# bjg-gh/style_transfer_visualizer

Hardware: AMD Instinct MI355X
Metric: optimization steps/sec at 512² and 1024², 1/2/4/8 MI355X (higher is better)
Workload: dtype bf16; 1 GPU; single 512x512 image per GPU, L-BFGS (max_iter=1, history 100), VGG19 bf16 storage / fp32 accumulate, fp32 Gram, --no-video (BASELINE.json configs[1]); weights: synthetic He-scaled; size=512, images=1, init_method=random, parallelism=replicas x1 (independent images), lbfgs_history_prefill_steps=95, world_size=1

## Files before the change

### style_transfer_visualizer_amd/csrc/conv_igemm_kernel.h

```cpp
#pragma once
#include <type_traits>
#include <utility>

#include "stv_common.h"
#include "conv_args.h"
#include "conv_tiles.h"

#ifndef STV_STAMP
#define STV_STAMP(k) do {} while (0)
#endif
#ifndef STV_DIAG
#define STV_DIAG 0
#endif

#ifndef STV_HOLD_LAST
#define STV_HOLD_LAST 1
#endif
#ifndef STV_X_AUX
#define STV_X_AUX 0
#endif
#ifndef STV_STORE_AUX
#define STV_STORE_AUX 0
#endif

extern thread_local const void* g_stv_next_w;
extern thread_local uint32_t g_stv_next_w_bytes;

namespace {


template <typename T, int TH_, int BN_, int WM_, int WN_, int TAPS_, int KS_ = 1, int NBUF_ = 3, bool M16_ = false,
          bool X3_ = false>
struct Cfg {
  static constexpr bool X3 = X3_;
  static constexpr bool M16 = M16_;
  using Elem = T;
  static constexpr int TH = TH_, BN = BN_, WM = WM_, WN = WN_, TAPS = TAPS_;
  static constexpr int NWAVES = WM_ * WN_;
  static constexpr int KS = KS_;
  static constexpr int GT = 64 * NWAVES;
  static constexpr int TW = 32;
  static constexpr int KB = 32;
  static constexpr int CK = KB / (int)sizeof(T);
  static constexpr int HALO = (TAPS == 9) ? 1 : 0;
  static constexpr int ND = (TAPS == 9) ? 3 : 1;
  static constexpr int IN_H = TH + 2 * HALO, IN_W = TW + 2 * HALO;
  static constexpr int IN_PIX = IN_H * IN_W;
  static constexpr int W_ROWS = TAPS * BN;
  static constexpr int MT = TH / WM;
  static constexpr int NT = BN / WN / 32;
  static constexpr int AROWS = MT + 2 * HALO;
  static constexpr bool BIG = MT * NT >= 8;
  static constexpr int THREADS = GT * KS;
  static constexpr int IN_PIECES = (IN_PIX * 2 + 63) / 64;
  static constexpr int W_PIECES = (W_ROWS * 2 + 63) / 64;
  static constexpr int PIECES = IN_PIECES + W_PIECES;
  static constexpr int PPW = (PIECES + NWAVES - 1) / NWAVES;
  static constexpr int IN_BYTES = IN_PIECES * 1024;
  static constexpr int SPARE_OFF = PIECES * 1024;
  static constexpr int STAGE_BYTES = SPARE_OFF + 1024;
  static constexpr int NBUF = NBUF_;
  static constexpr int BM = TH * TW;
  static constexpr int CS = BN + 4;
  static constexpr int C_BYTES = BM * CS * 4;
  static constexpr int RING_BYTES = NBUF * KS * STAGE_BYTES;
  static constexpr int LDS_BYTES = (KS == 1 || RING_BYTES > C_BYTES) ? RING_BYTES : C_BYTES;
  static_assert(NWAVES * KS == 4 || NWAVES * KS == 8, "4 or 8 waves per workgroup");
  static_assert(KS == 1 || KS == 2, "K split");
  static_assert(NBUF >= 2 && NBUF <= 6, "ring depth");
  static_assert(!M16 || (NBUF == 4 && sizeof(T) == 2), "16x16x32 main loop: bf16, two pairs of stage slots");
  static_assert(!X3 || (sizeof(T) == 4 && !M16), "split-bf16 products: fp32 storage, 32x32 main loop");
  static_assert(TH % WM == 0 && BN % (WN * 32) == 0, "tile split");
  static_assert(BN % 16 == 0, "swizzle period");
  static_assert(LDS_BYTES <= 160 * 1024, "LDS budget");
};

template <typename T> struct Frag;
template <> struct Frag<bf16_t> { using type = bf16x8v; };
template <> struct Frag<float> { using type = f32x4; };

template <typename T>
__device__ __forceinline__ void mma(const typename Frag<T>::type& a,
                                    const typename Frag<T>::type& b, f32x16& acc);
template <>
__device__ __forceinline__ void mma<bf16_t>(const bf16x8v& a, const bf16x8v& b, f32x16& acc) {
  acc = __builtin_amdgcn_mfma_f32_32x32x16_bf16(a, b, acc, 0, 0, 0);
}
template <>
__device__ __forceinline__ void mma<float>(const f32x4& a, const f32x4& b, f32x16& acc) {
#pragma unroll
  for (int j = 0; j < 4; ++j) acc = __builtin_amdgcn_mfma_f32_32x32x2f32(a[j], b[j], acc, 0, 0, 0);
}

struct X3Act { bf16x8v p, q; };

__device__ __forceinline__ float bf16_hi_part(float x, uint32_t& bits) {
  bits = (uint32_t)f32_to_bf16(x);
  return __uint_as_float(bits << 16);
}
__device__ __forceinline__ void split4(f32x4 v, uint32_t (&hi)[2], uint32_t (&lo)[2]) {
#pragma unroll
  for (int i = 0; i < 2; ++i) {
    uint32_t b0, b1;
    const float h0 = bf16_hi_part(v[2 * i], b0), h1 = bf16_hi_part(v[2 * i + 1], b1);
    const float r0 = __builtin_isfinite(h0) ? v[2 * i] - h0 : 0.0f;
    const float r1 = __builtin_isfinite(h1) ? v[2 * i + 1] - h1 : 0.0f;
    hi[i] = b0 | (b1 << 16);
    lo[i] = pack_bf16x2(r0, r1);
  }
}
__device__ __forceinline__ X3Act split_act(f32x4 v) {
  uint32_t hi[2], lo[2];
  split4(v, hi, lo);
  const u32x4 p = {hi[0], hi[1], hi[0], hi[1]}, q = {lo[0], lo[1], 0u, 0u};
  return X3Act{__builtin_bit_cast(bf16x8v, p), __builtin_bit_cast(bf16x8v, q)};
}
__device__ __forceinline__ bf16x8v split_w(f32x4 v) {
  uint32_t hi[2], lo[2];
  split4(v, hi, lo);
  const u32x4 w = {hi[0], hi[1], lo[0], lo[1]};
  return __builtin_bit_cast(bf16x8v, w);
}
__device__ __forceinline__ void mma_any(const f32x4& b, const f32x4& a, f32x16& acc) { mma<float>(b, a, acc); }
__device__ __forceinline__ void mma_any(const bf16x8v& b, const bf16x8v& a, f32x16& acc) { mma<bf16_t>(b, a, acc); }
__device__ __forceinline__ void mma_any(const bf16x8v& w, const X3Act& a, f32x16& acc) {
  acc = __builtin_amdgcn_mfma_f32_32x32x16_bf16(w, a.p, acc, 0, 0, 0);
  acc = __builtin_amdgcn_mfma_f32_32x32x16_bf16(w, a.q, acc, 0, 0, 0);
}

template <typename T>
struct Phase {
  const T* x;
  const T* w;
  int cin;
  bool w_blocked;
};
struct Geom {
  int H, W, cout, x0, y0, n0;
  int lane, wave, grp, wm, wn, r, h;
};

template <typename C, bool RELU>
__device__ __forceinline__ void conv_mainloop(const Phase<typename C::Elem>& ph, const Geom& gm, char* smem,
                                              f32x16 (&acc)[C::MT][C::NT]) {
  using T = typename C::Elem;
  using FragT = typename Frag<T>::type;
  using AFrag = std::conditional_t<C::X3, X3Act, FragT>;
  using BFrag = std::conditional_t<C::X3, bf16x8v, FragT>;
  using lds_ptr = __attribute__((address_space(3))) void*;
  constexpr int kVec = elem_traits<T>::kVec;
  const int lane = gm.lane, wave = gm.wave, grp = gm.grp, wm = gm.wm, wn = gm.wn, r = gm.r, h = gm.h;
  const int x0 = gm.x0, y0 = gm.y0, n0 = gm.n0;
  const int nchunks = ph.cin / C::CK;
  constexpr uint32_t kOob = 0x80000000u;
  const int x_bytes = gm.H * gm.W * ph.cin * (int)sizeof(T);
  const int w_bytes = C::TAPS * gm.cout * ph.cin * (int)sizeof(T);
  const int w_stride = ph.w_blocked ? gm.cout * C::KB : C::KB;
  auto piece_id = [&](int j) { return j * C::NWAVES + wave; };
  uint32_t p_off[C::PPW];
#pragma unroll
  for (int j = 0; j < C::PPW; ++j) {
    const int g = piece_id(j);
    if (g < C::IN_PIECES) {
      const int v = g * 64 + lane;
      const int pix = v >> 1;
      const int half = (v & 1) ^ ((pix >> 3) & 1);
      const int py = pix / C::IN_W, px = pix - py * C::IN_W;
      const int gy = y0 + py - C::HALO, gx = x0 + px - C::HALO;
      const bool ok = pix < C::IN_PIX && gy >= 0 && gy < gm.H && gx >= 0 && gx < gm.W;
      p_off[j] = ok ? (uint32_t)(((gy * gm.W + gx) * ph.cin + half * kVec) * (int)sizeof(T)) : kOob;
    } else {
      const int v = (g - C::IN_PIECES) * 64 + lane;
      const int row = v >> 1;
      const int half = (v & 1) ^ ((row >> 3) & 1);
      const int tap = row / C::BN, nn = row - tap * C::BN;
      const bool ok = row < C::W_ROWS && (n0 + nn) < gm.cout;
      const int elem = ph.w_blocked ? ((tap * nchunks * gm.cout + n0 + nn) * C::CK + half * kVec)
                                 : ((tap * gm.cout + n0 + nn) * ph.cin + half * kVec);
      p_off[j] = ok ? (uint32_t)(elem * (int)sizeof(T)) : kOob;
    }
  }
  const int nrounds = (nchunks + C::KS - 1) / C::KS;
  char* const ring = smem + grp * (C::NBUF * C::STAGE_BYTES);
  auto dma = [&](int j, int l, char* buf) {
    const int g = piece_id(j);
    const int stage = l * C::KS + grp;
    const bool in = g < C::IN_PIECES;
    const bool live = g < C::PIECES && stage < nchunks && !(STV_DIAG & 1);
    const __amdgpu_buffer_rsrc_t rs = __builtin_amdgcn_make_buffer_rsrc(
        const_cast<T*>(in ? ph.x : ph.w), 0, live ? (in ? x_bytes : w_bytes) : 0, 0x00020000);
    char* dst = buf + (g < C::PIECES ? g * 1024 : C::SPARE_OFF);
    if (STV_X_AUX != 0 && in) __builtin_amdgcn_raw_ptr_buffer_load_lds(rs, (lds_ptr)dst, 16, p_off[j], stage * C::KB, 0, STV_X_AUX);
    else __builtin_amdgcn_raw_ptr_buffer_load_lds(rs, (lds_ptr)dst, 16, p_off[j], stage * (in ? C::KB : w_stride), 0, 0);
  };

  int a_addr[C::ND][C::AROWS];
#pragma unroll
  for (int dx = 0; dx < C::ND; ++dx)
#pragma unroll
    for (int j = 0; j < C::AROWS; ++j) {
      const int pix = (wm * C::MT + j) * C::IN_W + dx + r;
      a_addr[dx][j] = pix * C::KB + ((h ^ ((pix >> 3) & 1)) << 4);
    }
  const int b_lane = C::IN_BYTES + (wn * (C::NT * 32) + r) * C::KB + ((h ^ ((r >> 3) & 1)) << 4);

  constexpr int NSTEP = C::ND * C::ND;
  constexpr int NISS = (C::BIG && C::NBUF == 2 && NSTEP > 1) ? (NSTEP + 1) / 2 : NSTEP;
  constexpr int PER = (C::PPW + NISS - 1) / NISS;
  constexpr int PFB = (C::MT * C::NT >= 4) ? 2 : 3;

  constexpr bool BLOCKED = sizeof(T) == 4;
  constexpr int NHOLD = (BLOCKED || C::BIG) ? 0 : ((STV_HOLD_LAST < NSTEP) ? STV_HOLD_LAST : NSTEP);
  AFrag hold_a[NHOLD > 0 ? NHOLD : 1][C::MT];
  BFrag hold_b[NHOLD > 0 ? NHOLD : 1][C::NT];
#pragma unroll
  for (int q = 0; q < NHOLD; ++q) {
#pragma unroll
    for (int mt = 0; mt < C::MT; ++mt) hold_a[q][mt] = AFrag{};
#pragma unroll
    for (int nt = 0; nt < C::NT; ++nt) hold_b[q][nt] = BFrag{};
  }
  auto flush_held = [&]() {
#pragma unroll
    for (int q = 0; q < NHOLD; ++q)
#pragma unroll
      for (int mt = 0; mt < C::MT; ++mt)
#pragma unroll
        for (int nt = 0; nt < C::NT; ++nt) mma_any(hold_b[q][nt], hold_a[q][mt], acc[mt][nt]);
  };
  auto run_stage = [&](const char* cur, char* fill, int l) {
    AFrag af[2][C::AROWS];
    BFrag bf[PFB + 1][C::NT];
    f32x16 sacc[BLOCKED ? C::MT : 1][BLOCKED ? C::NT : 1];
    if constexpr (BLOCKED) {
#pragma unroll
      for (int mt = 0; mt < C::MT; ++mt)
#pragma unroll
        for (int nt = 0; nt < C::NT; ++nt)
#pragma unroll
          for (int i = 0; i < 16; ++i) sacc[mt][nt][i] = 0.0f;
    }
    auto load_a = [&](int dx, int j, int set) {
      const FragT v = *reinterpret_cast<const FragT*>(cur + a_addr[dx][j]);
      if constexpr (C::X3) af[set][j] = split_act(RELU ? relu_frag(v, 0u) : v);
      else af[set][j] = RELU ? relu_frag(v, 0u) : v;
    };
    auto load_b = [&](int step) {
      const int tap = (step % C::ND) * C::ND + step / C::ND;
#pragma unroll
      for (int nt = 0; nt < C::NT; ++nt) {
        const char* src = cur + b_lane + (tap * C::BN + nt * 32) * C::KB;
        if constexpr (C::X3 && C::TAPS == 9)
          bf[step % (PFB + 1)][nt] = *reinterpret_cast<const bf16x8v*>(src);
        else if constexpr (C::X3)
          bf[step % (PFB + 1)][nt] = split_w(*reinterpret_cast<const f32x4*>(src));
        else
          bf[step % (PFB + 1)][nt] = *reinterpret_cast<const FragT*>(src);
      }
    };
    load_b(0);
#pragma unroll
    for (int j = 0; j < C::AROWS; ++j) load_a(0, j, 0);
#pragma unroll
    for (int q = 1; q < PFB; ++q)
      if (q < NSTEP) load_b(q);
    if (NHOLD > 0) {
      __builtin_amdgcn_sched_barrier(0);
      flush_held();
      __builtin_amdgcn_sched_barrier(0);
    }
#pragma unroll
    for (int step = 0; step < NSTEP; ++step) {
      const int dx = step / C::ND, dy = step % C::ND;
      if (step + PFB < NSTEP) load_b(step + PFB);
      if (dx + 1 < C::ND) {
#pragma unroll
        for (int j = 0; j < C::AROWS; ++j)
          if ((j < (C::AROWS + 1) / 2 ? 0 : 1) == dy) load_a(dx + 1, j, (dx + 1) & 1);
      }
#pragma unroll
      for (int k = step * PER; k < (step + 1) * PER; ++k)
        if (k < C::PPW) dma(k, l + C::NBUF - 1, fill);
      __builtin_amdgcn_sched_barrier(0);
      if (step >= NSTEP - NHOLD) {
        const int q = step - (NSTEP - NHOLD);
#pragma unroll
        for (int mt = 0; mt < C::MT; ++mt) hold_a[q][mt] = af[dx & 1][mt + dy];
#pragma unroll
        for (int nt = 0; nt < C::NT; ++nt) hold_b[q][nt] = bf[step % (PFB + 1)][nt];
      } else {
#pragma unroll
        for (int mt = 0; mt < C::MT; ++mt)
#pragma unroll
          for (int nt = 0; nt < C::NT; ++nt) {
            if constexpr (BLOCKED) mma_any(bf[step % (PFB + 1)][nt], af[dx & 1][mt + dy], sacc[mt][nt]);
            else mma_any(bf[step % (PFB + 1)][nt], af[dx & 1][mt + dy], acc[mt][nt]);
          }
      }
      __builtin_amdgcn_sched_barrier(0);
    }
    if constexpr (BLOCKED) {
#pragma unroll
      for (int mt = 0; mt < C::MT; ++mt)
#pragma unroll
        for (int nt = 0; nt < C::NT; ++nt)
#pragma unroll
          for (int i = 0; i < 16; ++i) acc[mt][nt][i] += sacc[mt][nt][i];
    }
    wait_vmcnt<(C::NBUF - 2) * C::PPW>();
    __builtin_amdgcn_s_barrier();
  };

#if defined(STV_PRIO_HALF)
  if (C::NWAVES * C::KS == 8 && (int)(threadIdx.x >> 8) == 1) __builtin_amdgcn_s_setprio(1);
#endif
#pragma unroll
  for (int rnd = 0; rnd + 1 < C::NBUF; ++rnd)
#pragma unroll
    for (int k = 0; k < C::PPW; ++k) dma(k, rnd, ring + rnd * C::STAGE_BYTES);
  wait_vmcnt<(C::NBUF - 2) * C::PPW>();
  __builtin_amdgcn_s_barrier();
  STV_STAMP(1);

  int c = 0;
  for (; c + C::NBUF <= nrounds; c += C::NBUF) {
#pragma unroll
    for (int k = 0; k < C::NBUF; ++k)
      run_stage(ring + k * C::STAGE_BYTES, ring + ((k + C::NBUF - 1) % C::NBUF) * C::STAGE_BYTES, c + k);
  }
#pragma unroll
  for (int k = 0; k + 1 < C::NBUF; ++k)
    if (c + k < nrounds) run_stage(ring + k * C::STAGE_BYTES, ring + ((k + C::NBUF - 1) % C::NBUF) * C::STAGE_BYTES, c + k);
  if (NHOLD > 0) flush_held();
  wait_vmcnt<0>();
  __syncthreads();

}

template <typename C, bool RELU>
__device__ __forceinline__ void conv_mainloop16(const Phase<bf16_t>& ph, const Geom& gm, char* smem,
                                                f32x4 (&acc)[C::MT][2][C::NT][2]) {
  using T = bf16_t;
  using FragT = bf16x8v;
  using lds_ptr = __attribute__((address_space(3))) void*;
  constexpr int kVec = 8;
  const int lane = gm.lane, wave = gm.wave, grp = gm.grp, wm = gm.wm, wn = gm.wn;
  const int x0 = gm.x0, y0 = gm.y0, n0 = gm.n0;
  const int nchunks = ph.cin / C::CK;
  const int npairs = nchunks >> 1;
  constexpr uint32_t kOob = 0x80000000u;
  const int x_bytes = gm.H * gm.W * ph.cin * (int)sizeof(T);
  const int w_bytes = C::TAPS * gm.cout * ph.cin * (int)sizeof(T);
  const int w_stride = ph.w_blocked ? gm.cout * C::KB : C::KB;
  auto piece_id = [&](int j) { return j * C::NWAVES + wave; };
  uint32_t p_off[C::PPW];
#pragma unroll
  for (int j = 0; j < C::PPW; ++j) {
    const int g = piece_id(j);
    if (g < C::IN_PIECES) {
      const int v = g * 64 + lane;
      const int pix = v >> 1, half = v & 1;
      const int py = pix / C::IN_W, px = pix - py * C::IN_W;
      const int gy = y0 + py - C::HALO, gx = x0 + px - C::HALO;
      const bool ok = pix < C::IN_PIX && gy >= 0 && gy < gm.H && gx >= 0 && gx < gm.W;
      p_off[j] = ok ? (uint32_t)(((gy * gm.W + gx) * ph.cin + half * kVec) * (int)sizeof(T)) : kOob;
    } else {
      const int v = (g - C::IN_PIECES) * 64 + lane;
      const int row = v >> 1, half = v & 1;
      const int tap = row / C::BN, nn = row - tap * C::BN;
      const bool ok = row < C::W_ROWS && (n0 + nn) < gm.cout;
      const int elem = ph.w_blocked ? ((tap * nchunks * gm.cout + n0 + nn) * C::CK + half * kVec)
                                    : ((tap * gm.cout + n0 + nn) * ph.cin + half * kVec);
      p_off[j] = ok ? (uint32_t)(elem * (int)sizeof(T)) : kOob;
    }
  }
  const int nrounds = (npairs + C::KS - 1) / C::KS;
  char* const ring = smem + grp * (C::NBUF * C::STAGE_BYTES);
  constexpr int PAIR_BYTES = 2 * C::STAGE_BYTES;
  auto dma = [&](int k, int l, char* pair) {
    const int sub = k / C::PPW, j = k - sub * C::PPW;
    const int g = piece_id(j);
    const int stage = 2 * (l * C::KS + grp) + sub;
    const bool in = g < C::IN_PIECES;
    const bool live = g < C::PIECES && stage < nchunks && !(STV_DIAG & 1);
    const __amdgpu_buffer_rsrc_t rs = __builtin_amdgcn_make_buffer_rsrc(
        const_cast<T*>(in ? ph.x : ph.w), 0, live ? (in ? x_bytes : w_bytes) : 0, 0x00020000);
    char* dst = pair + sub * C::STAGE_BYTES + (g < C::PIECES ? g * 1024 : C::SPARE_OFF);
    if (STV_X_AUX != 0 && in) __builtin_amdgcn_raw_ptr_buffer_load_lds(rs, (lds_ptr)dst, 16, p_off[j], stage * C::KB, 0, STV_X_AUX);
    else __builtin_amdgcn_raw_ptr_buffer_load_lds(rs, (lds_ptr)dst, 16, p_off[j], stage * (in ? C::KB : w_stride), 0, 0);
  };

  const int px = lane & 15, kg = (lane >> 4) & 1, sub = lane >> 5;
  const int a_lane = sub * C::STAGE_BYTES + ((wm * C::MT) * C::IN_W + px) * C::KB + kg * 16;
  const int b_lane = sub * C::STAGE_BYTES + C::IN_BYTES + (wn * (C::NT * 32) + px) * C::KB + kg * 16;

  constexpr int U = C::ND * C::AROWS;
  constexpr int NISS = (U >= 2) ? U / 2 : 1;
  constexpr int PER = (2 * C::PPW + NISS - 1) / NISS;
  constexpr int PFP = (U >= 3) ? 2 : 1;

  auto run_round = [&](const char* cur, char* fill, int l) {
    FragT wf[2][C::ND][C::NT][2];
    FragT pf[PFP + 1][2];
    auto load_w = [&](int dx, int dy) {
      const int tap = dy * C::ND + dx;
#pragma unroll
      for (int nt = 0; nt < C::NT; ++nt)
#pragma unroll
        for (int cb = 0; cb < 2; ++cb)
          wf[dx & 1][dy][nt][cb] = *reinterpret_cast<const FragT*>(cur + b_lane + (tap * C::BN + nt * 32 + cb * 16) * C::KB);
    };
    auto load_p = [&](int u) {
      const int dx = u / C::AROWS, j = u - dx * C::AROWS;
#pragma unroll
      for (int pb = 0; pb < 2; ++pb) {
        const FragT v = *reinterpret_cast<const FragT*>(cur + a_lane + (j * C::IN_W + dx + pb * 16) * C::KB);
        pf[u % (PFP + 1)][pb] = RELU ? relu_frag(v, 0u) : v;
      }
    };
#pragma unroll
    for (int dy = 0; dy < C::ND; ++dy) load_w(0, dy);
#pragma unroll
    for (int u = 0; u < PFP; ++u)
      if (u < U) load_p(u);
#pragma unroll
    for (int u = 0; u < U; ++u) {
      const int dx = u / C::AROWS, j = u - dx * C::AROWS;
      if (u + PFP < U) load_p(u + PFP);
      if (dx + 1 < C::ND && j < C::ND) load_w(dx + 1, j);
#pragma unroll
      for (int k = u * PER; k < (u + 1) * PER; ++k)
        if (u < NISS && k < 2 * C::PPW) dma(k, l + 1, fill);
      __builtin_amdgcn_sched_barrier(0);
#pragma unroll
      for (int dy = 0; dy < C::ND; ++dy) {
        const int mt = j - dy;
        if (mt < 0 || mt >= C::MT) continue;
#pragma unroll
        for (int nt = 0; nt < C::NT; ++nt)
#pragma unroll
          for (int cb = 0; cb < 2; ++cb)
#pragma unroll
            for (int pb = 0; pb < 2; ++pb)
              acc[mt][pb][nt][cb] = __builtin_amdgcn_mfma_f32_16x16x32_bf16(wf[dx & 1][dy][nt][cb], pf[u % (PFP + 1)][pb],
                                                                            acc[mt][pb][nt][cb], 0, 0, 0);
      }
      __builtin_amdgcn_sched_barrier(0);
    }
    wait_vmcnt<0>();
    __builtin_amdgcn_s_barrier();
  };

#pragma unroll
  for (int k = 0; k < 2 * C::PPW; ++k) dma(k, 0, ring);
  wait_vmcnt<0>();
  __builtin_amdgcn_s_barrier();
  STV_STAMP(1);
  int l = 0;
  for (; l + 2 <= nrounds; l += 2) {
    run_round(ring, ring + PAIR_BYTES, l);
    run_round(ring + PAIR_BYTES, ring, l + 1);
  }
  if (l < nrounds) run_round(ring, ring + PAIR_BYTES, l);
  wait_vmcnt<0>();
  __syncthreads();
}

template <typename C>
__device__ __forceinline__ void acc16_to_acc32(const f32x4 (&a16)[C::MT][2][C::NT][2], f32x16 (&acc)[C::MT][C::NT], bool add) {
#pragma unroll
  for (int mt = 0; mt < C::MT; ++mt)
#pragma unroll
    for (int nt = 0; nt < C::NT; ++nt)
#pragma unroll
      for (int cb = 0; cb < 2; ++cb)
#pragma unroll
        for (int e = 0; e < 4; ++e) {
          const auto s1 = __builtin_amdgcn_permlane16_swap(__float_as_uint(a16[mt][0][nt][cb][e]), __float_as_uint(a16[mt][1][nt][cb][e]), false, false);
          const auto s2 = __builtin_amdgcn_permlane32_swap(s1[0], s1[1], false, false);
          const float v0 = __uint_as_float(s2[0]), v1 = __uint_as_float(s2[1]);
          if (add) {
            acc[mt][nt][8 * cb + e] += v0;
            acc[mt][nt][8 * cb + 4 + e] += v1;
          } else {
            acc[mt][nt][8 * cb + e] = v0;
            acc[mt][nt][8 * cb + 4 + e] = v1;
          }
        }
}

template <typename C, bool RELU>
__device__ __forceinline__ void run_phase(const Phase<typename C::Elem>& ph, const Geom& gm, char* smem,
                                          f32x16 (&acc)[C::MT][C::NT], bool add) {
  if constexpr (C::M16) {
    f32x4 a16[C::MT][2][C::NT][2];
#pragma unroll
    for (int mt = 0; mt < C::MT; ++mt)
#pragma unroll
      for (int pb = 0; pb < 2; ++pb)
#pragma unroll
        for (int nt = 0; nt < C::NT; ++nt)
#pragma unroll
          for (int cb = 0; cb < 2; ++cb) a16[mt][pb][nt][cb] = f32x4{0.0f, 0.0f, 0.0f, 0.0f};
    conv_mainloop16<C, RELU>(ph, gm, smem, a16);
    acc16_to_acc32<C>(a16, acc, add);
  } else {
    conv_mainloop<C, RELU>(ph, gm, smem, acc);
  }
}

template <typename C, bool RELU>
__global__ __launch_bounds__(C::THREADS) void conv_igemm_kernel(ConvArgs a) {
#if defined(__HIP_DEVICE_COMPILE__)
  using T = typename C::Elem;
  extern __shared__ __attribute__((aligned(16))) char smem[];

  const int tid = threadIdx.x;
  const int lane = tid & 63;
  const int wave_wg = __builtin_amdgcn_readfirstlane(tid >> 6) & (C::NWAVES * C::KS - 1);
  const int grp = wave_wg / C::NWAVES;
  const int wave = wave_wg % C::NWAVES;
  const int wm = wave / C::WN, wn = wave % C::WN;
  const int r = lane & 31, h = lane >> 5;

  const int tiles_x = (a.W + C::TW - 1) / C::TW;
  const int ntiles = tiles_x * ((a.H + C::TH - 1) / C::TH);
  const int ny = (a.cout + C::BN - 1) / C::BN;
  const int blk = (int)blockIdx.x;
  const int grp8 = blk / (8 * ny), within = blk - grp8 * (8 * ny);
  const int left = ntiles - grp8 * 8;
  const int span = left < 8 ? left : 8;
  const int tile = grp8 * 8 + within % span;
  const int yb = within / span;
  const int tile_x = tile % tiles_x;
  const int tile_y = tile / tiles_x;
  const int x0 = tile_x * C::TW, y0 = tile_y * C::TH;
  const int n0 = yb * C::BN;

  const T* __restrict__ xin = static_cast<const T*>(a.x);
  const T* __restrict__ wgt = static_cast<const T*>(a.w);
  const bool w_blocked = (a.flags & STV_W_BLOCKED) != 0;
  STV_STAMP(0);
  const __amdgpu_buffer_rsrc_t rs_b = __builtin_amdgcn_make_buffer_rsrc(
      const_cast<float*>(a.bias), 0, a.bias != nullptr ? a.cout * 4 : 0, 0x00020000);
  f32x4 bias_v[C::NT][4];
  auto load_bias = [&]() {
#pragma unroll
    for (int nt = 0; nt < C::NT; ++nt)
#pragma unroll
      for (int j = 0; j < 4; ++j) {
        const int nn = n0 + wn * (C::NT * 32) + nt * 32 + 8 * j + 4 * (lane >> 5);
        const u32x4 t = __builtin_amdgcn_raw_buffer_load_b128(rs_b, (uint32_t)(nn * 4), 0, 0);
#pragma unroll
        for (int e = 0; e < 4; ++e) bias_v[nt][j][e] = __uint_as_float(t[e]);
      }
  };
  if constexpr (!C::BIG) load_bias();

  f32x16 acc[C::MT][C::NT];
#pragma unroll
  for (int mt = 0; mt < C::MT; ++mt)
#pragma unroll
    for (int nt = 0; nt < C::NT; ++nt)
#pragma unroll
      for (int i = 0; i < 16; ++i) acc[mt][nt][i] = 0.0f;

  constexpr uint32_t kOob = 0x80000000u;
  const Geom geom{a.H, a.W, a.cout, x0, y0, n0, lane, wave, grp, wm, wn, r, h};
  run_phase<C, RELU>(Phase<T>{xin, wgt, a.cin, w_blocked}, geom, smem, acc, false);
  STV_STAMP(2);

  bool mask_done = false;
  if constexpr (C::TAPS == 9) {
    if (a.x2 != nullptr) {
      if (a.flags & STV_MASK) {
        const int ref_bytes = a.H * a.W * a.cout * (int)sizeof(T);
        const __amdgpu_buffer_rsrc_t rs_m = __builtin_amdgcn_make_buffer_rsrc(const_cast<void*>(a.ref), 0, ref_bytes, 0x00020000);
#pragma unroll
        for (int mt = 0; mt < C::MT; ++mt) {
          const int gy = y0 + wm * C::MT + mt, gx = x0 + r;
          const bool pok = gy < a.H && gx < a.W;
#pragma unroll
          for (int nt = 0; nt < C::NT; ++nt)
#pragma unroll
            for (int j = 0; j < 4; ++j) {
              const int nn = n0 + wn * (C::NT * 32) + nt * 32 + 8 * j + 4 * h;
              const uint32_t off = (pok && nn < a.cout) ? (uint32_t)((((gy * a.W + gx) * a.cout) + nn) * (int)sizeof(T)) : kOob;
              if constexpr (sizeof(T) == 4) {
                const u32x4 m = __builtin_amdgcn_raw_buffer_load_b128(rs_m, off, 0, 0);
#pragma unroll
                for (int e = 0; e < 4; ++e) acc[mt][nt][4 * j + e] = (__uint_as_float(m[e]) > 0.0f) ? acc[mt][nt][4 * j + e] : 0.0f;
              } else {
                const auto m = __builtin_amdgcn_raw_buffer_load_b64(rs_m, off, 0, 0);
                keep_where_bf16_positive(acc[mt][nt], 4 * j, m[0], m[1]);
              }
            }
        }
        mask_done = true;
      }
      using C1 = Cfg<T, C::TH, C::BN, C::WM, C::WN, 1, C::KS, C::NBUF, C::M16, C::X3>;
      static_assert(C1::RING_BYTES <= C::LDS_BYTES, "the 1x1 pass reuses the 3x3 ring");
      const Phase<T> ph2{static_cast<const T*>(a.x2), static_cast<const T*>(a.w2), a.cin2, false};
      run_phase<C1, false>(ph2, geom, smem, acc, true);
    }
  }

  if constexpr (C::BIG) load_bias();
  const __amdgpu_buffer_rsrc_t rs_pf = __builtin_amdgcn_make_buffer_rsrc(const_cast<void*>(a.pf), 0, (int)a.pf_bytes, 0x00020000);
  const uint32_t pf_word = __builtin_amdgcn_raw_buffer_load_b32(rs_pf, ((uint32_t)blockIdx.x * C::THREADS + (uint32_t)tid) * 128u, 0, 0);

  const bool relu_out = (a.flags & STV_RELU_OUT) != 0;
  const bool do_mask = (a.flags & STV_MASK) != 0 && !mask_done && a.route_out == nullptr;
  const bool do_acc = (a.flags & STV_ACCUM) != 0;
  const int out_bytes = a.H * a.W * a.cout * (int)sizeof(T);
  const __amdgpu_buffer_rsrc_t rs_y = __builtin_amdgcn_make_buffer_rsrc(a.y, 0, a.y != nullptr ? out_bytes : 0, 0x00020000);
  const __amdgpu_buffer_rsrc_t rs_ref = __builtin_amdgcn_make_buffer_rsrc(
      const_cast<void*>(a.ref), 0, do_mask ? out_bytes : 0, 0x00020000);
  const __amdgpu_buffer_rsrc_t rs_old = __builtin_amdgcn_make_buffer_rsrc(a.y, 0, do_acc ? out_bytes : 0, 0x00020000);
  const bool route = sizeof(T) == 2 && a.route_out != nullptr;
  const bool route_mask = (a.flags & STV_MASK) != 0 && route;
  const __amdgpu_buffer_rsrc_t rs_ridx = __builtin_amdgcn_make_buffer_rsrc(
      const_cast<void*>(a.route_idx), 0, route ? a.H * a.W * a.cout : 0, 0x00020000);
  const __amdgpu_buffer_rsrc_t rs_route = __builtin_amdgcn_make_buffer_rsrc(a.route_out, 0, route ? 4 * out_bytes : 0, 0x00020000);

  if (C::KS == 2) {
    float* cs = reinterpret_cast<float*>(smem);
    auto c_tile = [&](auto mode) {
#pragma unroll
      for (int mt = 0; mt < C::MT; ++mt)
#pragma unroll
        for (int nt = 0; nt < C::NT; ++nt)
#pragma unroll
          for (int i = 0; i < 16; ++i) {
            const int row = (wm * C::MT + mt) * 32 + (i & 3) + 8 * (i >> 2) + 4 * h;
            const int col = wn * (C::NT * 32) + nt * 32 + r;
            if (decltype(mode)::value == 0) cs[row * C::CS + col] = acc[mt][nt][i];
            else acc[mt][nt][i] += cs[row * C::CS + col];
          }
    };
    if (grp == 1) c_tile(std::integral_constant<int, 0>{});
    __syncthreads();
    if (grp == 0) c_tile(std::integral_constant<int, 1>{});
  }
  STV_STAMP(3);

  if (grp == 0) {
    auto emit = [&](auto&& val, auto&& pix_off, const __amdgpu_buffer_rsrc_t& rs_out, int MTN, bool masked, bool accum) {
#pragma unroll
      for (int mt = 0; mt < C::MT; ++mt) {
        if (mt >= MTN) continue;
        const uint32_t poff = pix_off(mt);
#pragma unroll
        for (int nt = 0; nt < C::NT; ++nt) {
          const int nb = n0 + wn * (C::NT * 32) + nt * 32;
          if constexpr (sizeof(T) == 4) {
#pragma unroll
            for (int j = 0; j < 4; ++j) {
              const int nn = nb + 8 * j + 4 * h;
              const uint32_t off = (poff != kOob && nn < a.cout) ? poff + (uint32_t)(nn * 4) : kOob;
              float v[4];
#pragma unroll
              for (int e = 0; e < 4; ++e) {
                v[e] = val(mt, nt, 4 * j + e) + bias_v[nt][j][e];
                if (relu_out) v[e] = fmaxf(v[e], 0.0f);
              }
              if (masked) {
                const u32x4 m = __builtin_amdgcn_raw_buffer_load_b128(rs_ref, off, 0, 0);
#pragma unroll
                for (int e = 0; e < 4; ++e) v[e] = (__uint_as_float(m[e]) > 0.0f) ? v[e] : 0.0f;
              }
              if (accum) {
                const u32x4 o = __builtin_amdgcn_raw_buffer_load_b128(rs_old, off, 0, 0);
#pragma unroll
                for (int e = 0; e < 4; ++e) v[e] += __uint_as_float(o[e]);
              }
              const u32x4 out = {__float_as_uint(v[0]), __float_as_uint(v[1]), __float_as_uint(v[2]), __float_as_uint(v[3])};
              __builtin_amdgcn_raw_buffer_store_b128(out, rs_out, off, 0, 0);
            }
          } else {
            uint32_t px[4], py[4];
#pragma unroll
            for (int j = 0; j < 4; ++j) {
              float v[4];
#pragma unroll
              for (int e = 0; e < 4; ++e) {
                v[e] = val(mt, nt, 4 * j + e) + bias_v[nt][j][e];
                if (relu_out) v[e] = fmaxf(v[e], 0.0f);
              }
              if (accum) {
                const int nn = nb + 8 * j + 4 * h;
                const uint32_t off = (poff != kOob && nn < a.cout) ? poff + (uint32_t)(nn * 2) : kOob;
                if (masked) {
                  const auto m = __builtin_amdgcn_raw_buffer_load_b64(rs_ref, off, 0, 0);
                  keep_where_bf16_positive(v, 0, m[0], m[1]);
                }
                const auto o = __builtin_amdgcn_raw_buffer_load_b64(rs_old, off, 0, 0);
                v[0] += __uint_as_float(o[0] << 16);
                v[1] += __uint_as_float(o[0] & 0xFFFF0000u);
                v[2] += __uint_as_float(o[1] << 16);
                v[3] += __uint_as_float(o[1] & 0xFFFF0000u);
              }
              px[j] = pack_bf16x2(v[0], v[1]);
              py[j] = pack_bf16x2(v[2], v[3]);
            }
#pragma unroll
            for (int jp = 0; jp < 4; jp += 2) {
              const auto sx = __builtin_amdgcn_permlane32_swap(px[jp], px[jp + 1], false, false);
              const auto sy = __builtin_amdgcn_permlane32_swap(py[jp], py[jp + 1], false, false);
              u32x4 out = {sx[0], sy[0], sx[1], sy[1]};
              const int nn = nb + 8 * jp + 8 * h;
              const uint32_t off = (poff != kOob && nn < a.cout) ? poff + (uint32_t)(nn * 2) : kOob;
              if (masked && !accum) {
                typedef __attribute__((ext_vector_type(8))) short s16x8;
                const s16x8 m = __builtin_bit_cast(s16x8, __builtin_amdgcn_raw_buffer_load_b128(rs_ref, off, 0, 0));
                const s16x8 keep = (s16x8)(m > (s16x8)(short)0);
                out = __builtin_bit_cast(u32x4, __builtin_bit_cast(s16x8, out) & keep);
              }
              if (route) {
                const uint32_t ioff = off != kOob ? (off >> 1) : kOob;
                const auto ib = __builtin_amdgcn_raw_buffer_load_b64(rs_ridx, ioff, 0, 0);
                const int gy = y0 + wm * C::MT + mt, gx = x0 + r;
                const uint32_t base = (uint32_t)((((2 * gy) * (2 * a.W) + 2 * gx) * a.cout + nn) * 2);
#pragma unroll
                for (int pos = 0; pos < 4; ++pos) {
                  uint32_t keep[4];
#pragma unroll
                  for (int half = 0; half < 2; ++half) {
                    const uint32_t want = route_mask ? 0x01010101u * (uint32_t)(pos | 4) : 0x01010101u * (uint32_t)pos;
                    const uint32_t x = (route_mask ? ib[half] : (ib[half] & 0x03030303u)) ^ want;
                    const uint32_t hit = ((~(x + 0x7F7F7F7Fu) & 0x80808080u) >> 7) * 0xFFu;
                    keep[2 * half] = __builtin_amdgcn_perm(hit, hit, 0x01010000u);
                    keep[2 * half + 1] = __builtin_amdgcn_perm(hit, hit, 0x03030202u);
                  }
                  const u32x4 v = {out[0] & keep[0], out[1] & keep[1], out[2] & keep[2], out[3] & keep[3]};
                  const uint32_t o2 = off != kOob ? base + (uint32_t)((((pos >> 1) * 2 * a.W + (pos & 1)) * a.cout) * 2) : kOob;
                  __builtin_amdgcn_raw_buffer_store_b128(v, rs_route, o2, 0, STV_STORE_AUX);
                }
              } else {
                __builtin_amdgcn_raw_buffer_store_b128(out, rs_out, off, 0, STV_STORE_AUX);
              }
            }
          }
        }
      }
    };
    auto full_off = [&](int mt) -> uint32_t {
      const int gy = y0 + wm * C::MT + mt, gx = x0 + r;
      if (STV_DIAG & 2) return kOob;
      return (gy < a.H && gx < a.W) ? (uint32_t)(((gy * a.W + gx) * a.cout) * (int)sizeof(T)) : kOob;
    };
    if (!((a.flags & STV_POOL_ONLY) && a.pool != nullptr && C::MT % 2 == 0))
      emit([&](int mt, int nt, int i) { return acc[mt][nt][i]; }, full_off, rs_y, C::MT, do_mask, do_acc);

    if constexpr (C::MT % 2 == 0) if (a.pool != nullptr) {
      const int Hp = a.H >> 1, Wp = a.W >> 1;
      const __amdgpu_buffer_rsrc_t rs_p = __builtin_amdgcn_make_buffer_rsrc(a.pool, 0, Hp * Wp * a.cout * (int)sizeof(T), 0x00020000);
      auto pooled = [&](int mp, int nt, int i) -> float {
        const float v = fmaxf(acc[2 * mp][nt][i], acc[2 * mp + 1][nt][i]);
        return fmaxf(v, __shfl_xor(v, 1, 64));
      };
      auto pool_off = [&](int mp) -> uint32_t {
        const int gyp = ((y0 + wm * C::MT) >> 1) + mp, gxp = (x0 + r) >> 1;
        return ((r & 1) == 0 && gyp < Hp && gxp < Wp) ? (uint32_t)(((gyp * Wp + gxp) * a.cout) * (int)sizeof(T)) : kOob;
      };
      emit([&](int mp, int nt, int i) { return pooled(mp < C::MT / 2 ? mp : 0, nt, i); }, pool_off, rs_p, C::MT / 2, false, false);

      if (a.pool_idx != nullptr) {
        const __amdgpu_buffer_rsrc_t rs_i = __builtin_amdgcn_make_buffer_rsrc(a.pool_idx, 0, Hp * Wp * a.cout, 0x00020000);
        auto stored = [&](float v) -> float {
          if (relu_out) v = fmaxf(v, 0.0f);
          if constexpr (sizeof(T) == 2) v = bf16_to_f32(f32_to_bf16(v));
          return v;
        };
        auto right = [](float v) -> float {
          return __builtin_bit_cast(float, __builtin_amdgcn_update_dpp(0, __builtin_bit_cast(int, v), 0xB1, 0xF, 0xF, false));
        };
#pragma unroll
        for (int mp = 0; mp < C::MT / 2; ++mp) {
          const int gyp = ((y0 + wm * C::MT) >> 1) + mp, gxp = (x0 + r) >> 1;
          const bool pix_ok = (r & 1) == 0 && gyp < Hp && gxp < Wp;
#pragma unroll
          for (int nt = 0; nt < C::NT; ++nt) {
            const int nb = n0 + wn * (C::NT * 32) + nt * 32;
#pragma unroll
            for (int j = 0; j < 4; ++j) {
              uint32_t word = 0;
#pragma unroll
              for (int e = 0; e < 4; ++e) {
                const float tl = stored(acc[2 * mp][nt][4 * j + e] + bias_v[nt][j][e]);
                const float bl = stored(acc[2 * mp + 1][nt][4 * j + e] + bias_v[nt][j][e]);
                const float tr = right(tl), br = right(bl);
                float best = tl;
                uint32_t code = 0;
                if (tr > best) { best = tr; code = 1; }
                if (bl > best) { best = bl; code = 2; }
                if (br > best) { best = br; code = 3; }
                if (best > 0.0f) code |= 4;
                word |= code << (8 * e);
              }
              const int nn = nb + 8 * j + 4 * h;
              const uint32_t off = (pix_ok && nn < a.cout) ? (uint32_t)((gyp * Wp + gxp) * a.cout + nn) : kOob;
              __builtin_amdgcn_raw_buffer_store_b32(word, rs_i, off, 0, 0);
            }
          }
        }
      }
    }
  }
  STV_STAMP(4);
  asm volatile("" ::"v"(pf_word));
#endif
}

template <typename C>
int launch_cfg(const ConvArgs& a_in, hipStream_t st) {
  ConvArgs a = a_in;
  a.pf = g_stv_next_w;
  a.pf_bytes = g_stv_next_w ? g_stv_next_w_bytes : 0;
  g_stv_next_w = nullptr;
  g_stv_next_w_bytes = 0;
  const bool relu = (a.flags & STV_RELU_IN) != 0;
  const void* fn = relu ? reinterpret_cast<const void*>(&conv_igemm_kernel<C, true>)
                        : reinterpret_cast<const void*>(&conv_igemm_kernel<C, false>);
  if (stv_set_max_lds(fn, C::LDS_BYTES) != STV_OK) return STV_ERR_LAUNCH;
  const int tiles = ceil_div(a.W, C::TW) * ceil_div(a.H, C::TH);
  const int blocks = tiles * ceil_div(a.cout, C::BN);
  dim3 grid(blocks);
  if (relu) hipLaunchKernelGGL((conv_igemm_kernel<C, true>), grid, dim3(C::THREADS), C::LDS_BYTES, st, a);
  else hipLaunchKernelGGL((conv_igemm_kernel<C, false>), grid, dim3(C::THREADS), C::LDS_BYTES, st, a);
  STV_CHECK_LAUNCH();
  return STV_OK;
}

template <TileUnit UNIT, typename T, int TAPS, bool X3, int I>
bool launch_row(const ConvArgs& a, int cfg, hipStream_t st, int& rc) {
  constexpr Tile t = kTiles[I];
  if constexpr (t.unit == UNIT && (sizeof(T) == 2 || tile_serves_f32(I))) {
    if (cfg == I) {
      rc = launch_cfg<Cfg<T, t.TH, t.BN, t.WM, t.WN, TAPS, t.KS, t.NBUF, t.M16, X3>>(a, st);
      return true;
    }
  }
  return false;
}
template <TileUnit UNIT, typename T, int TAPS, bool X3, int... I>
int launch_rows(const ConvArgs& a, int cfg, hipStream_t st, std::integer_sequence<int, I...>) {
  int rc = STV_ERR_ARG;
  (void)(launch_row<UNIT, T, TAPS, X3, I>(a, cfg, st, rc) || ...);
  return rc;
}
template <TileUnit UNIT, typename T, int TAPS, bool X3 = false>
int launch_tile(const ConvArgs& a, int cfg, hipStream_t st) {
  return launch_rows<UNIT, T, TAPS, X3>(a, cfg, st, std::make_integer_sequence<int, kNumCfg>{});
}

}
```

Before: 1190 steps/s.

## Defer fused ReLU on activation fragments to overlap with MFMA issue

In the conv implicit-GEMM mainloops, the ReLU that was applied at LDS load time is now applied in place just before use and placed between MFMA groups. Empty asm fences keep the compiler from hoisting it back to the load. For bf16 multi-buffered configs, a third activation fragment set is added so loads run two dx columns ahead while the previous set is clamped. This is meant to stop the VALU clamp from stalling on LDS load latency and to hide it behind matrix ops, at the cost of extra VGPRs that may reduce occupancy or cause spills.

```diff
diff --git a/style_transfer_visualizer_amd/csrc/conv_igemm_kernel.h b/style_transfer_visualizer_amd/csrc/conv_igemm_kernel.h
--- a/style_transfer_visualizer_amd/csrc/conv_igemm_kernel.h
+++ b/style_transfer_visualizer_amd/csrc/conv_igemm_kernel.h
@@ -140,6 +140,16 @@
   int lane, wave, grp, wm, wn, r, h;
 };
 
+template <typename F>
+__device__ __forceinline__ void relu_in_place(F& f) {
+  if (STV_DIAG & 4) return;
+  u32x4 t = __builtin_bit_cast(u32x4, f);
+  asm volatile("" : "+v"(t));
+  t = __builtin_bit_cast(u32x4, relu_frag(__builtin_bit_cast(F, t), 0u));
+  asm volatile("" : "+v"(t));
+  f = __builtin_bit_cast(F, t);
+}
+
 template <typename C, bool RELU>
 __device__ __forceinline__ void conv_mainloop(const Phase<typename C::Elem>& ph, const Geom& gm, char* smem,
                                               f32x16 (&acc)[C::MT][C::NT]) {
@@ -228,8 +238,10 @@
 #pragma unroll
         for (int nt = 0; nt < C::NT; ++nt) mma_any(hold_b[q][nt], hold_a[q][mt], acc[mt][nt]);
   };
+  constexpr bool SHADOW = RELU && sizeof(T) == 2 && C::NBUF != 2;
+  constexpr int NSET = SHADOW ? 3 : 2;
   auto run_stage = [&](const char* cur, char* fill, int l) {
-    AFrag af[2][C::AROWS];
+    AFrag af[NSET][C::AROWS];
     BFrag bf[PFB + 1][C::NT];
     f32x16 sacc[BLOCKED ? C::MT : 1][BLOCKED ? C::NT : 1];
     if constexpr (BLOCKED) {
@@ -240,10 +252,17 @@
 #pragma unroll
           for (int i = 0; i < 16; ++i) sacc[mt][nt][i] = 0.0f;
     }
-    auto load_a = [&](int dx, int j, int set) {
+    auto load_a = [&](int dx, int j) {
       const FragT v = *reinterpret_cast<const FragT*>(cur + a_addr[dx][j]);
-      if constexpr (C::X3) af[set][j] = split_act(RELU ? relu_frag(v, 0u) : v);
-      else af[set][j] = RELU ? relu_frag(v, 0u) : v;
+      if constexpr (C::X3) af[dx % NSET][j] = split_act(RELU ? relu_frag(v, 0u) : v);
+      else af[dx % NSET][j] = (RELU && !SHADOW) ? relu_frag(v, 0u) : v;
+    };
+    auto relu_rows = [&](int dx, int j0, int j1) {
+      if constexpr (SHADOW) {
+#pragma unroll
+        for (int j = 0; j < C::AROWS; ++j)
+          if (j >= j0 && j < j1) relu_in_place(af[dx % NSET][j]);
+      }
     };
     auto load_b = [&](int step) {
       const int tap = (step % C::ND) * C::ND + step / C::ND;
@@ -260,10 +279,14 @@
     };
     load_b(0);
 #pragma unroll
-    for (int j = 0; j < C::AROWS; ++j) load_a(0, j, 0);
+    for (int j = 0; j < C::AROWS; ++j) load_a(0, j);
 #pragma unroll
     for (int q = 1; q < PFB; ++q)
       if (q < NSTEP) load_b(q);
+    if constexpr (SHADOW && C::ND > 1) {
+#pragma unroll
+      for (int j = 0; j < C::AROWS; ++j) load_a(1, j);
+    }
     if (NHOLD > 0) {
       __builtin_amdgcn_sched_barrier(0);
       flush_held();
@@ -273,10 +296,15 @@
     for (int step = 0; step < NSTEP; ++step) {
       const int dx = step / C::ND, dy = step % C::ND;
       if (step + PFB < NSTEP) load_b(step + PFB);
-      if (dx + 1 < C::ND) {
+      if constexpr (SHADOW) {
+        if (dy == 0 && dx + 2 < C::ND) {
+#pragma unroll
+          for (int j = 0; j < C::AROWS; ++j) load_a(dx + 2, j);
+        }
+      } else if (dx + 1 < C::ND) {
 #pragma unroll
         for (int j = 0; j < C::AROWS; ++j)
-          if ((j < (C::AROWS + 1) / 2 ? 0 : 1) == dy) load_a(dx + 1, j, (dx + 1) & 1);
+          if ((j < (C::AROWS + 1) / 2 ? 0 : 1) == dy) load_a(dx + 1, j);
       }
 #pragma unroll
       for (int k = step * PER; k < (step + 1) * PER; ++k)
@@ -284,18 +312,25 @@
       __builtin_amdgcn_sched_barrier(0);
       if (step >= NSTEP - NHOLD) {
         const int q = step - (NSTEP - NHOLD);
-#pragma unroll
-        for (int mt = 0; mt < C::MT; ++mt) hold_a[q][mt] = af[dx & 1][mt + dy];
+        if (step == 0) relu_rows(0, 0, C::MT);
+#pragma unroll
+        for (int mt = 0; mt < C::MT; ++mt) hold_a[q][mt] = af[dx % NSET][mt + dy];
 #pragma unroll
         for (int nt = 0; nt < C::NT; ++nt) hold_b[q][nt] = bf[step % (PFB + 1)][nt];
       } else {
 #pragma unroll
-        for (int mt = 0; mt < C::MT; ++mt)
+        for (int mt = 0; mt < C::MT; ++mt) {
+          if (step == 0) relu_rows(0, mt, mt + 1);
 #pragma unroll
           for (int nt = 0; nt < C::NT; ++nt) {
-            if constexpr (BLOCKED) mma_any(bf[step % (PFB + 1)][nt], af[dx & 1][mt + dy], sacc[mt][nt]);
-            else mma_any(bf[step % (PFB + 1)][nt], af[dx & 1][mt + dy], acc[mt][nt]);
+            if constexpr (BLOCKED) mma_any(bf[step % (PFB + 1)][nt], af[dx % NSET][mt + dy], sacc[mt][nt]);
+            else mma_any(bf[step % (PFB + 1)][nt], af[dx % NSET][mt + dy], acc[mt][nt]);
           }
+        }
+      }
+      if constexpr (SHADOW) {
+        if (dy + 1 < C::ND) relu_rows(dx, C::MT + dy, C::MT + dy + 1);
+        if (dy + 1 == C::ND && dx + 1 < C::ND) relu_rows(dx + 1, 0, C::MT);
       }
       __builtin_amdgcn_sched_barrier(0);
     }
@@ -413,9 +448,13 @@
     auto load_p = [&](int u) {
       const int dx = u / C::AROWS, j = u - dx * C::AROWS;
 #pragma unroll
-      for (int pb = 0; pb < 2; ++pb) {
-        const FragT v = *reinterpret_cast<const FragT*>(cur + a_lane + (j * C::IN_W + dx + pb * 16) * C::KB);
-        pf[u % (PFP + 1)][pb] = RELU ? relu_frag(v, 0u) : v;
+      for (int pb = 0; pb < 2; ++pb)
+        pf[u % (PFP + 1)][pb] = *reinterpret_cast<const FragT*>(cur + a_lane + (j * C::IN_W + dx + pb * 16) * C::KB);
+    };
+    auto clamp_p = [&](int u) {
+      if constexpr (RELU) {
+#pragma unroll
+        for (int pb = 0; pb < 2; ++pb) relu_in_place(pf[u % (PFP + 1)][pb]);
       }
     };
 #pragma unroll
@@ -432,6 +471,7 @@
       for (int k = u * PER; k < (u + 1) * PER; ++k)
         if (u < NISS && k < 2 * C::PPW) dma(k, l + 1, fill);
       __builtin_amdgcn_sched_barrier(0);
+      if (u == 0) clamp_p(0);
 #pragma unroll
       for (int dy = 0; dy < C::ND; ++dy) {
         const int mt = j - dy;
@@ -445,6 +485,7 @@
               acc[mt][pb][nt][cb] = __builtin_amdgcn_mfma_f32_16x16x32_bf16(wf[dx & 1][dy][nt][cb], pf[u % (PFP + 1)][pb],
                                                                             acc[mt][pb][nt][cb], 0, 0, 0);
       }
+      if (u + 1 < U) clamp_p(u + 1);
       __builtin_amdgcn_sched_barrier(0);
     }
     wait_vmcnt<0>();
```

After: 1189 steps/s. Within noise of the previous version (-0.1%).
